# 10258392511/InverseProblemWithDiffusionModel

Hardware: AMD Instinct MI355X
Metric: ALD reconstructions/sec (128x128 complex, R=40, 4-coil) (higher is better)
Workload: dtype f32 (convolutions: operands as two fp16 pieces = 22 significand bits + 2 signs, three fp16 MFMAs per product, fp32 accumulate; every image scaled into fp16's range by an exact power of two from its producer's per-image maxima: any fp32 input, DESIGN.md 4.2); 1 GPU; ACDC-style 128x128 complex SENSE R=40 4-coil ALD reconstruction, NCSNv2Deepest ngf=128 (94.1M params, seeded random init), sigma 348->0.01 x 2311 levels x 3 steps, L2Penalty, denoise; 14 posterior samples = 14 on rank 0 + 13 per further rank (the 105-sample / 8-GPU partition of BASELINE config 3); samples_total=14, samples_this_rank=14, parallelism=sample-sharded x1, hip_graph=True, state_finite=True

## Files before the change

include/ipdm.h:

```cpp
#ifndef IPDM_H
#define IPDM_H

#include <stdint.h>

#ifdef __cplusplus
extern "C" {
#endif

#define IPDM_OK 0
#define IPDM_EINVAL (-1)
#define IPDM_EUNSUPPORTED (-2)

#define IPDM_ACT_NONE 0
#define IPDM_ACT_ELU 1
#define IPDM_ACT_RELU 2
#define IPDM_ACT_LRELU02 3
#define IPDM_ACT_SWISH 4
#define IPDM_ACT_COPY 5

#define IPDM_AMAX_WAYS 8
#define IPDM_AMAX_SLOT 128

#define IPDM_ABI_VERSION 4
int ipdm_abi_version(void);
// ... 190 lines not shown
int ipdm_conv2d_wino_bx3_stats_f32(const float* x, const void* U, const float* bias, const float* residual, float* out,
                                   float* out_act, int act_out, int B, int Cin, int Cout, int H, int W, int dilation,
                                   int pool2, float* stats, const ipdm_conv_ext_t* ext, void* stream);
int ipdm_absmax_f32(const float* x, float* amax , int n_images,
                    int64_t per_image, void* stream);
int64_t ipdm_conv_hx2_weight_bytes(int Cout, int Cin, int k);
int ipdm_conv_hx2_pack_weight(const float* w , void* packed, int Cout,
                              int Cin, int k, void* stream);
int ipdm_conv2d_hx2_f32(const float* x, const void* packed, const float* bias, const float* coef, int act,
                        const float* residual, float* out, float* out_act, int act_out,
                        int B, int Cin, int Cout, int H, int W, int k, int dilation, const ipdm_conv_ext_t* ext, void* stream);
int ipdm_conv3d_hx2_f32(const float* x, const void* packed, const float* bias, const float* coef, int act,
                        const float* residual, float* out, float* out_act, int act_out,
                        int B, int Cin, int Cout, int D, int H, int W, int k, int dilation, const ipdm_conv_ext_t* ext, void* stream);
int ipdm_conv_hx2_splitk_f32(const float* x, const void* packed, const float* bias, const float* coef, int act,
                             const float* residual, float* out, float* out_act, int act_out,
                             int B, int Cin, int Cout, int D, int H, int W, int k, int dilation, int volume, int ksplit,
                             float* work, const ipdm_conv_ext_t* ext, void* stream);
int64_t ipdm_conv_wino_hx2_weight_bytes(int Cout, int Cin);
int ipdm_conv_wino_hx2_pack_weight(const float* w , void* U, int Cout, int Cin, void* stream);
int ipdm_conv2d_wino_hx2_f32(const float* x, const void* U, const float* bias, const float* residual, float* out,
                             float* out_act, int act_out, int B, int Cin, int Cout, int H, int W, int dilation,
                             int pool2, const ipdm_conv_ext_t* ext, void* stream);
int64_t ipdm_conv_wino1d_weight_bytes(int Cout, int Cin);
int ipdm_conv_wino1d_pack_weight(const float* w , void* U, int Cout, int Cin, void* stream);
int ipdm_conv2d_wino1d_supported(int Cin, int Cout, int H, int W);
int64_t ipdm_conv_wino1d_weight_bytes3d(int Cout, int Cin);
int ipdm_conv_wino1d_pack_weight3d(const float* w, void* U, int Cout, int Cin, void* stream);
int ipdm_conv3d_wino1d_supported(int Cin, int Cout, int D, int H, int W);
int ipdm_conv3d_wino1d_f32(const float* x, const void* U, const float* bias, const float* residual, float* out,
                           float* out_act, int act_out, int B, int Cin, int Cout, int D, int H, int W,
                           const ipdm_conv_ext_t* ext, void* stream);
int ipdm_conv2d_wino1d_f32(const float* x, const void* U, const float* bias, const float* coef, int act,
                           const float* residual, float* out, float* out_act, int act_out, int B, int Cin, int Cout, int H,
                           int W, int pool2, const ipdm_conv_ext_t* ext, void* stream);
int ipdm_conv2d_wino1d_stats_partials(int Cin, int Cout, int H, int W);
int ipdm_conv2d_wino1d_stats_f32(const float* x, const void* U, const float* bias, const float* coef, int act,
                                 const float* residual, float* out, float* out_act, int act_out, int B, int Cin, int Cout,
                                 int H, int W, int pool2, float* stats, const ipdm_conv_ext_t* ext, void* stream);
int ipdm_conv2d_wino_hx2_splitk_f32(const float* x, const void* U, const float* bias, const float* residual, float* out,
                                    float* out_act, int act_out, int B, int Cin, int Cout, int H, int W, int dilation,
                                    int ksplit, float* work, const ipdm_conv_ext_t* ext, void* stream);
int ipdm_conv2d_wino_hx2_stats_f32(const float* x, const void* U, const float* bias, const float* residual, float* out,
                                   float* out_act, int act_out, int B, int Cin, int Cout, int H, int W, int dilation,
                                   int pool2, float* stats, const ipdm_conv_ext_t* ext, void* stream);
int ipdm_instnorm_plus_coef_partials_f32(const float* partials, int P, const float* alpha, const float* gamma,
// ... 35 lines not shown
```

inverseproblemwithdiffusionmodel_amd/_lib.py:

```python
import ctypes
import os

import torch
from ctypes import c_char_p, c_float, c_int, c_int64, c_uint64, c_void_p


class ConvExt(ctypes.Structure):
    _fields_ = [("in_amax", c_void_p), ("bias_bstride", c_int), ("out_scale", c_float), ("res_second", c_int),
                ("out_amax", c_void_p), ("act_amax", c_void_p)]


_HERE = os.path.dirname(os.path.abspath(__file__))
LIB_PATH = os.environ.get("IPDM_LIB") or os.path.join(_HERE, "libipdm.so")

P = c_void_p

SIGNATURES = {
    "ipdm_abi_version": [],
    "ipdm_build_arch": [],
    "ipdm_upfirdn2d_f32": [P, P, P] + [c_int] * 14 + [P],
    "ipdm_fused_bias_act_f32": [P, P, P, P, c_int64, c_int, c_int, c_int, c_int, c_float, c_float, P],
    "ipdm_upfirdn2d_f16": [P, P, P] + [c_int] * 14 + [P],
    "ipdm_upfirdn2d_f64": [P, P, P] + [c_int] * 14 + [P],
    "ipdm_fused_bias_act_f16": [P, P, P, P, c_int64, c_int, c_int, c_int, c_int, c_float, c_float, P],
# ... 59 lines not shown
    "ipdm_conv2d_wino_bx3_stats_partials": [c_int, c_int, c_int, c_int, c_int, c_int],
    "ipdm_conv2d_wino_bx3_splitk": [c_int, c_int, c_int, c_int, c_int],
    "ipdm_conv2d_wino_bx3_splitk_f32": [P, P, P, P, P, P, c_int, c_int, c_int, c_int, c_int, c_int, c_int, c_int, P, P, P],
    "ipdm_conv2d_wino_bx3_stats_f32": [P, P, P, P, P, P, c_int, c_int, c_int, c_int, c_int, c_int, c_int, c_int, P, P, P],
    "ipdm_conv_hx2_weight_bytes": [c_int, c_int, c_int],
    "ipdm_conv_hx2_pack_weight": [P, P, c_int, c_int, c_int, P],
    "ipdm_absmax_f32": [P, P, c_int, c_int64, P],
    "ipdm_conv2d_hx2_f32": [P, P, P, P, c_int, P, P, P, c_int] + [c_int] * 7 + [P, P],
    "ipdm_conv3d_hx2_f32": [P, P, P, P, c_int, P, P, P, c_int] + [c_int] * 8 + [P, P],
    "ipdm_conv_hx2_splitk_f32": [P, P, P, P, c_int, P, P, P, c_int] + [c_int] * 10 + [P, P, P],
    "ipdm_conv_wino_hx2_weight_bytes": [c_int, c_int],
    "ipdm_conv_wino1d_weight_bytes": [c_int, c_int],
    "ipdm_conv_wino1d_pack_weight": [P, P, c_int, c_int, P],
    "ipdm_conv2d_wino1d_supported": [c_int, c_int, c_int, c_int],
    "ipdm_conv_wino1d_weight_bytes3d": [c_int, c_int],
    "ipdm_conv_wino1d_pack_weight3d": [P, P, c_int, c_int, P],
    "ipdm_conv3d_wino1d_supported": [c_int, c_int, c_int, c_int, c_int],
    "ipdm_conv3d_wino1d_f32": [P, P, P, P, P, P, c_int, c_int, c_int, c_int, c_int, c_int, c_int, P, P],
    "ipdm_conv2d_wino1d_f32": [P, P, P, P, c_int, P, P, P, c_int, c_int, c_int, c_int, c_int, c_int, c_int, P, P],
    "ipdm_conv2d_wino1d_stats_partials": [c_int, c_int, c_int, c_int],
    "ipdm_conv2d_wino1d_stats_f32": [P, P, P, P, c_int, P, P, P, c_int, c_int, c_int, c_int, c_int, c_int, c_int, P, P, P],
    "ipdm_conv_wino_hx2_pack_weight": [P, P, c_int, c_int, P],
    "ipdm_conv2d_wino_hx2_f32": [P, P, P, P, P, P, c_int, c_int, c_int, c_int, c_int, c_int, c_int, c_int, P, P],
    "ipdm_conv2d_wino_hx2_splitk_f32": [P, P, P, P, P, P, c_int, c_int, c_int, c_int, c_int, c_int, c_int, c_int, P, P, P],
    "ipdm_conv2d_wino_hx2_stats_f32": [P, P, P, P, P, P, c_int, c_int, c_int, c_int, c_int, c_int, c_int, c_int, P, P, P],
    "ipdm_instnorm_plus_coef_partials_f32": [P, c_int, P, P, P, P, c_int, c_int, c_int, P, P],
    "ipdm_cond_instnorm_plus_coef_partials_f32": [P, c_int, P, P, c_int, c_int, P, c_int, c_int, c_int, P, P],
    "ipdm_zero_insert2_f32": [P, P, c_int, c_int, c_int, P],
    "ipdm_subsample2_f32": [P, P, c_int, c_int, c_int, c_int, c_int, c_int, c_int, P],
    "ipdm_in_prelu_fwd_f32": [P, P, P, P, P, c_int, c_int, c_float, P],
    "ipdm_in_prelu_bwd_f32": [P, P, P, P, P, c_int, c_int, P],
    "ipdm_seg_loglh_grad_f32": [P, P, P, c_int, c_int, c_int64, P],
    "ipdm_axpy_sched_f32": [P, P, P, c_int64, P, c_float, c_int64, P],
    "ipdm_magnitude_c64": [P, P, c_int64, P],
    "ipdm_posterior_moments_c64": [P, P, c_int, c_int64, P],
    "ipdm_tv_c64": [P, P, c_int, c_int, c_int, P],
    "ipdm_tv_grad_c64": [P, P, c_int, c_int, c_int, P],
    "ipdm_nrmse_f32": [P, P, P, c_int, c_int64, c_int, P],
    "ipdm_ssim_f32": [P, P, P, c_int, c_int, c_int, c_int, ctypes.c_double, P],
}
_RESTYPES = {"ipdm_build_arch": c_char_p, "ipdm_fft2c_workspace_bytes": c_int64, "ipdm_sense_workspace_bytes": c_int64, "ipdm_conv_bx3_weight_bytes": c_int64,
             "ipdm_conv_wino_bx3_weight_bytes": c_int64, "ipdm_conv_hx2_weight_bytes": c_int64,
             "ipdm_conv_wino_hx2_weight_bytes": c_int64, "ipdm_conv_wino1d_weight_bytes": c_int64, "ipdm_conv_wino1d_weight_bytes3d": c_int64}

IPDM_EINVAL = -1
IPDM_EUNSUPPORTED = -2
# ... 39 lines not shown
```

inverseproblemwithdiffusionmodel_amd/csrc/conv_wino_bx3.hip:

```cpp
#include "conv_kernel.h"

namespace ipdm_conv {

namespace {

constexpr int X_KC = 16;
constexpr int X_CO = 64;
constexpr int X_TX = 16, X_TY = 4;
constexpr int X_TILES = X_TX * X_TY;
constexpr int X_V_ELEMS = 16 * X_KC * X_TILES;
constexpr int X_RR = 2 * X_TY + 2, X_RC = 2 * X_TX + 2;
constexpr int X_RCH = 384;
constexpr int X_R_ELEMS = 32 * 256;
constexpr size_t X_LDS_BYTES = (2 * (size_t)X_V_ELEMS + X_R_ELEMS) * sizeof(float);

__global__ __launch_bounds__(256) void wino_bx3_weight_kernel(const float* __restrict__ w, unsigned short* __restrict__ out,
                                                              int Cout, int Cin, int n_cc, int n_ct) {
  const float G[4][3] = {{1.f, 0.f, 0.f}, {0.5f, 0.5f, 0.5f}, {0.5f, -0.5f, 0.5f}, {0.f, 0.f, 1.f}};
  const int64_t total = (int64_t)16 * n_cc * n_ct * 512;
  for (int64_t i = (int64_t)blockIdx.x * 256 + threadIdx.x; i < total; i += (int64_t)gridDim.x * 256) {
    const int q = (int)(i & 7), r = (int)((i >> 3) & 31), h = (int)((i >> 8) & 1);
    const int64_t rest = i >> 9;
    const int ct = (int)(rest % n_ct);
    const int cc = (int)((rest / n_ct) % n_cc);
// ... 479 lines not shown
              const float e1 = a.act_out == IPDM_ACT_ELU ? fast_elu(y1v) : ipdm_act(y1v, a.act_out);
              amx_a = fmaxf(amx_a, fmaxf(fabsf(e0), fabsf(e1)));
              *reinterpret_cast<float2*>(a.out_act + o) = make_float2(e0, e1);
            }
          }
        }
      }
    }
  }
  if (a.amax_out) ipdm_amax_commit(amx_o, a.amax_out + (size_t)b * IPDM_AMAX_SLOT, wave);
  if (a.amax_act) ipdm_amax_commit(amx_a, a.amax_act + (size_t)b * IPDM_AMAX_SLOT, wave);
  if (a.dbg) {
    __builtin_amdgcn_s_waitcnt(0);
    const unsigned long long t3 = __builtin_amdgcn_s_memtime();
    if (tid == 0) {
      unsigned long long* d4 = a.dbg + (size_t)blockIdx.x * 4;
      d4[0] = t0; d4[1] = t1; d4[2] = t2; d4[3] = t3;
    }
  }
}


template <bool HX, int TX, int TY, bool CO_MAJOR, bool DMA4, bool POOL = false, bool STATS = false, bool KSP = false, bool POLY = false,
          bool CO32 = false>
__global__ __launch_bounds__(512) void conv_wino_bx3_wide_kernel(ConvArgs a, int total_tiles) {
  constexpr int NPC = HX ? 2 : 3;
  constexpr int FRAG = 64 * NPC;
  constexpr int NC = CO32 ? 1 : 2;
  static_assert(!CO32 || (HX && TX == 8 && TY == 8 && DMA4 && !POOL && !STATS && !KSP && !POLY), "CO32: the plain 8 x 8 form");
  static_assert(!POLY || (TX == 8 && TY == 8 && DMA4 && !POOL && !STATS && !KSP), "POLY: the 8 x 8 form, plain epilogue");
  constexpr int PPW = 24, PPH = 17;
  constexpr int QC = POLY ? PPW / 4 : TX / 2 + 2, RC4 = 4 * QC;
  constexpr int QN = POLY ? PPH * QC : (2 * TY + 2) * QC;
  constexpr int NI = (X_KC * QN + 63) / 64;
  static_assert(NI >= 24 && NI <= 32 && NI * 256 <= X_R_ELEMS, "quad image fits the raw stage; pieces 0..23 exist");
  constexpr bool WPRIV = HX && DMA4;
  static_assert(!WPRIV || 2 * QN <= 256, "a wave's two channels fit four DMA instructions");
  static_assert(TX * TY == X_TILES, "64 tiles per workgroup");
  constexpr int RC = 2 * TX + 2, RR = 2 * TY + 2;
  static_assert(RC * RR <= X_RCH, "raw region fits its LDS slot");
  extern __shared__ __align__(16) float lds[];
  unsigned long long t0 = 0, t1 = 0, t2 = 0;
  if (a.dbg) t0 = __builtin_amdgcn_s_memtime();
  const int tid = threadIdx.x;
  const int lane = tid & 63;
  const int wave = __builtin_amdgcn_readfirstlane(tid >> 6);
  const int h = lane >> 5, j = lane & 31;
  const int HW = a.H * a.W;
  const int n_cc = a.Cin / X_KC, n_ct = a.Cout / 32;
  const int n_chunks = KSP ? n_cc / a.ksplit : n_cc;
  const int p0 = 2 * wave;

  const int S = gridDim.x / 8;
  const int xcd = blockIdx.x % 8, slot = blockIdx.x / 8;
  const int q = total_tiles / 8, r8 = total_tiles % 8;
  const int x_start = xcd < r8 ? xcd * (q + 1) : r8 * (q + 1) + (xcd - r8) * q;
  const int x_end = x_start + q + (xcd < r8 ? 1 : 0);
#ifdef IPDM_WBX3_RUNS
  constexpr bool RUNS = true;
#else
  constexpr bool RUNS = false;
// ... 9 lines not shown
    Geo g;
    g.ks = 0;
    g.c0 = 0;
    int n_px = total_tiles / a.co_tiles;
    if constexpr (KSP) {
      g.ks = L % a.ksplit;
      L /= a.ksplit;
      n_px /= a.ksplit;
      g.c0 = g.ks * n_chunks;
    }
    g.co_tile = CO_MAJOR ? L / n_px : L % a.co_tiles;
    int t = CO_MAJOR ? L % n_px : L / a.co_tiles;
    const int tx = t % a.tiles_x;
    t /= a.tiles_x;
    g.y0 = (t % a.tiles_y) * (2 * TY);
    g.x0 = tx * (2 * TX);
    g.b = t / a.tiles_y;
    return g;
  };

  const __amdgpu_buffer_rsrc_t x_rsrc = __builtin_amdgcn_make_buffer_rsrc(
      const_cast<float*>(a.x), 0, (int)((size_t)a.B * a.Cin * HW * 4), 0x00020000);
  float* const rs = lds + 2 * X_V_ELEMS;
  const int mytile = tid & 63;

  int dma_off[DMA4 ? 4 : 6];
  int dma_b = 0;
  [[maybe_unused]] int dma_c0 = 0;
  auto dma_piece = [&](int k) { return wave + 8 * k < NI ? wave + 8 * k : wave + 8 * (k - 1); };
  auto set_dma_geo = [&](const Geo& g) {
    dma_b = g.b;
    if constexpr (KSP) dma_c0 = g.c0;
    if constexpr (DMA4) {
#pragma unroll
      for (int k = 0; k < 4; ++k) {
        const int e = (WPRIV ? k : dma_piece(k)) * 64 + lane;
        const int cl = e / QN, qq = e - cl * QN;
        const int cin = WPRIV ? 2 * wave + cl : cl;
        const int rr = qq / QC, qc = qq - rr * QC;
        const int gy = POLY ? (rr < 16 ? rr : -1) : g.y0 - 1 + rr, gx0 = g.x0 - 4 + 4 * qc;
        const bool ok = e < (WPRIV ? 2 : X_KC) * QN && gy >= 0 && gy < a.H && gx0 >= 0 && gx0 < a.W;
        dma_off[k] = ok ? (cin * HW + gy * a.W + gx0) * 4 : 0x40000000;
      }
    } else {
#pragma unroll
      for (int k = 0; k < 6; ++k) {
        const int e = k * 64 + lane;
        const int rr = e / RC, c = e - rr * RC;
        const int gy = g.y0 - 1 + rr, gx = g.x0 - 1 + c;
        const bool ok = e < RR * RC && gy >= 0 && gy < a.H && gx >= 0 && gx < a.W;
        dma_off[k] = ok ? (gy * a.W + gx) * 4 : 0x40000000;
      }
    }
  };
  auto issue_dma = [&](int chunk) {
    if constexpr (KSP) chunk += dma_c0;
    if constexpr (DMA4) {
      [[maybe_unused]] const int soff = (int)(((size_t)dma_b * a.Cin + chunk * X_KC) * HW * 4);
#pragma unroll
      for (int k = 0; k < 4; ++k) {
#if defined(__HIP_DEVICE_COMPILE__)
        __builtin_amdgcn_raw_ptr_buffer_load_lds(
            x_rsrc, (__attribute__((address_space(3))) void*)(rs + (WPRIV ? wave * 4 + k : dma_piece(k)) * 256), 16, dma_off[k],
            soff, 0, 0);
#endif
      }
    } else {
#pragma unroll
      for (int cl = 0; cl < 2; ++cl) {
        const int kc = 2 * wave + cl;
        const int soff = (int)(((size_t)dma_b * a.Cin + chunk * X_KC + kc) * HW * 4);
#pragma unroll
        for (int k = 0; k < 6; ++k)
          __builtin_amdgcn_raw_ptr_buffer_load_lds(x_rsrc, (__attribute__((address_space(3))) void*)(rs + kc * X_RCH + k * 64), 4,
                                                   dma_off[k], soff, 0, 0);
      }
    }
  };
  float dreg[16];
  const int pd = POLY ? a.dil : 1;
  auto tile_origin = [&](int tl, int& py, int& px) {
    const int tws = a.W / (2 * pd), ths = a.H / (2 * pd);
    const int txx = tl % tws;
    int r = tl / tws;
    const int tyy = r % ths;
    r /= ths;
    py = pd * (2 * tyy) + r / pd;
    px = pd * (2 * txx) + r % pd;
  };
  [[maybe_unused]] int prow[4], pcol[4];
  if constexpr (POLY) {
    int py, px;
    tile_origin(mytile, py, px);
#pragma unroll
    for (int e = 0; e < 4; ++e) {
      const int gy = py + pd * (e - 1), gx = px + pd * (e - 1);
      prow[e] = (gy >= 0 && gy < a.H ? gy : 16) * PPW;
      pcol[e] = gx >= 0 && gx < a.W ? gx + 4 : 0;
    }
  }
  const int r_lane = DMA4 ? (2 * (mytile / TX)) * RC4 + 2 * (mytile % TX) + 2 : (2 * (mytile / TX)) * RC + 2 * (mytile % TX);
  auto read_patch_to = [&](float (&dreg)[16], int kc) {
    if constexpr (POLY) {
      const float* rp = WPRIV ? rs + wave * 1024 + (kc & 1) * (QN * 4) : rs + kc * (QN * 4);
#pragma unroll
      for (int rr = 0; rr < 4; ++rr)
#pragma unroll
        for (int cc = 0; cc < 4; ++cc) dreg[rr * 4 + cc] = rp[prow[rr] + pcol[cc]];
    } else if constexpr (DMA4) {
      const float* rp = (WPRIV ? rs + wave * 1024 + (kc & 1) * (QN * 4) : rs + kc * (QN * 4)) + r_lane;
      const int txl = mytile % TX;
// ... 62 lines not shown
  [[maybe_unused]] float hx_in = HX_WINO_PRESCALE, hx_out = 1.f;
  auto hx_scales_of = [&](int b, float& s_in, float& s_out) {
    s_in = HX_WINO_PRESCALE;
    s_out = 1.f;
    if constexpr (HX) {
      if (a.in_amax) {
        float sd, si;
        hx_dynamic_scale(ipdm_amax_read(a.in_amax + (size_t)b * IPDM_AMAX_SLOT), sd, si);
        s_in = HX_WINO_PRESCALE * sd;
        s_out = si;
      }
    }
  };
  auto store_pair = [&](float* st, const float (&va)[16], const float (&vb)[16], auto p_lo, auto p_hi) {
    unsigned* vs = reinterpret_cast<unsigned*>(st) + wave * X_TILES + mytile;
#pragma unroll
    for (int p = decltype(p_lo)::value; p < decltype(p_hi)::value; ++p) {
      unsigned hp, lp;
      split2_pk_scaled(va[p], vb[p], hx_in, hp, lp);
      vs[(p * 2 + 0) * (8 * X_TILES)] = hp;
      vs[(p * 2 + 1) * (8 * X_TILES)] = lp;
    }
  };
  auto stage_chunk = [&](float* st) {
    if constexpr (HX) {
      float va[16], vb[16];
      read_patch_to(va, 2 * wave);
      transform(va);
      read_patch_to(vb, 2 * wave + 1);
      transform(vb);
      store_pair(st, va, vb, std::integral_constant<int, 0>{}, std::integral_constant<int, 16>{});
    } else {
      read_patch(2 * wave);
      store_patch(st, 2 * wave);
      read_patch(2 * wave + 1);
      store_patch(st, 2 * wave + 1);
    }
  };

  const uint4* wq = reinterpret_cast<const uint4*>(a.wt);
  const size_t pos_stride = (size_t)n_cc * n_ct * FRAG;
  auto load_A = [&](uint4 (&fr)[NC][NPC], int p, int cc, int co_tile) {
    const uint4* base = wq + (size_t)p * pos_stride + ((size_t)cc * n_ct + co_tile * NC) * FRAG + lane;
#pragma unroll
    for (int c = 0; c < NC; ++c)
#pragma unroll
      for (int s = 0; s < NPC; ++s) fr[c][s] = base[c * FRAG + s * 64];
  };
  const int b_lane = (8 * h) * X_TILES + j;
  auto load_B = [&](float (&raw)[8], const float* cur, int pi, int tg) {
    const float* bp = cur + (p0 + pi) * (X_KC * X_TILES) + tg * 32 + b_lane;
#pragma unroll
    for (int qq = 0; qq < 8; ++qq) raw[qq] = bp[qq * X_TILES];
  };
  auto load_Bh = [&](uint4 (&fr)[2], const float* cur, int pi, int tg) {
    const unsigned* bp = reinterpret_cast<const unsigned*>(cur) + (p0 + pi) * (X_KC * X_TILES) + (4 * h) * X_TILES + tg * 32 + j;
#pragma unroll
    for (int s = 0; s < 2; ++s)
      fr[s] = make_uint4(bp[s * 8 * X_TILES], bp[(s * 8 + 1) * X_TILES], bp[(s * 8 + 2) * X_TILES], bp[(s * 8 + 3) * X_TILES]);
  };

  f32x16 acc[2][NC][2];
  auto zero_acc = [&]() {
#pragma unroll
    for (int i = 0; i < 4 * NC; ++i)
#pragma unroll
      for (int rr = 0; rr < 16; ++rr) acc[i / (2 * NC)][(i >> 1) % NC][i & 1][rr] = 0.f;
  };
  zero_acc();

  Geo cur_g = geo_of(tile);
  uint4 afr[2][NC][NPC];
  load_A(afr[0], p0, cur_g.c0, cur_g.co_tile);
  if constexpr (WPRIV) load_A(afr[1], p0 + 1, cur_g.c0, cur_g.co_tile);
  hx_scales_of(cur_g.b, hx_in, hx_out);
  set_dma_geo(cur_g);
  auto lds_barrier = [&]() {
    __builtin_amdgcn_sched_barrier(0);
    __builtin_amdgcn_s_waitcnt(0xC07F);
    __builtin_amdgcn_s_barrier();
    asm volatile("" ::: "memory");
    __builtin_amdgcn_sched_barrier(0);
  };
  issue_dma(0);
  __builtin_amdgcn_s_waitcnt(0);
  __syncthreads();
  stage_chunk(lds);
  __syncthreads();
  issue_dma(1);
  __builtin_amdgcn_s_waitcnt(0);
// ... 23 lines not shown
#define IPDM_TE(k)
#endif
  while (true) {
    const int next_tile = tile + t_step;
    const bool has_next = next_tile < t_end;
    const Geo next_g = geo_of(has_next ? next_tile : tile);
    for (int ch = 0; ch < n_chunks; ++ch, ++g) {
#ifdef IPDM_WBX3_TRACE
      const bool trace_now = g == n_chunks + 2;
#endif
      IPDM_TR(0);
      const float* cur = lds + (g & 1) * X_V_ELEMS;
      float* nxt = lds + ((g + 1) & 1) * X_V_ELEMS;
      const bool dma_next = ch + 2 >= n_chunks;
      const int dma_chunk = dma_next ? ch + 2 - n_chunks : ch + 2;
      if (ch + 2 == n_chunks) set_dma_geo(next_g);
      const bool a_next = ch + 1 >= n_chunks;
      const int a_chunk = a_next ? next_g.c0 : cur_g.c0 + ch + 1;
      const int a_cot = a_next ? next_g.co_tile : cur_g.co_tile;
      if constexpr (HX) {
        [[maybe_unused]] float unused_out;
        if (a_next && next_g.b != cur_g.b) hx_scales_of(next_g.b, hx_in, unused_out);
      }
      if constexpr (WPRIV) {
        uint4 bsh[2][2];
        float va[16], vb[16];
        __builtin_amdgcn_s_waitcnt(0x0F74);
        read_patch_to(va, 2 * wave);
        read_patch_to(vb, 2 * wave + 1);
        load_Bh(bsh[0], cur, 0, 0);
        __builtin_amdgcn_sched_barrier(0);
        __builtin_amdgcn_s_waitcnt(0xC07F);
        IPDM_TR(5);
        issue_dma(dma_chunk);
        __builtin_amdgcn_sched_barrier(0);
        static_for<4>([&](auto sc) {
          constexpr int st = decltype(sc)::value;
          constexpr int pi = st >> 1, tg = st & 1;
          if constexpr (st < 3) load_Bh(bsh[(st + 1) & 1], cur, (st + 1) >> 1, (st + 1) & 1);
          if constexpr (st == 0) transform(va);
          if constexpr (st == 1) transform(vb);
          if constexpr (st == 2) {
            store_pair(nxt, va, vb, std::integral_constant<int, 0>{}, std::integral_constant<int, 8>{});
            load_A(afr[0], p0, a_chunk, a_cot);
          }
          if constexpr (st == 3) store_pair(nxt, va, vb, std::integral_constant<int, 8>{}, std::integral_constant<int, 16>{});
          const f16x8 bh = __builtin_bit_cast(f16x8, bsh[st & 1][0]), bl = __builtin_bit_cast(f16x8, bsh[st & 1][1]);
// ... 151 lines not shown
    if (a.dbg) t2 = __builtin_amdgcn_s_memtime();

    float* ms = lds + ((g - 1) & 1) * X_V_ELEMS;
    IPDM_TE(0);
    const int etile = tid & 31, ecg = tid >> 5;
    const int co0 = cur_g.co_tile * (CO32 ? 32 : X_CO);
    constexpr int NR = POOL ? 1 : 2;
    constexpr bool AHEAD = TX == 16;
    float2 resv[AHEAD ? 2 : 1][2][NR];
    float biasv[AHEAD ? 2 : 1][2];
    [[maybe_unused]] float scalev[AHEAD ? 2 : 1][2];
    const float* const scale_p = HX ? reinterpret_cast<const float*>(wq + 16 * pos_stride) : a.wt;
    [[maybe_unused]] const int oH = POOL ? a.H >> 1 : a.H, oW = POOL ? a.W >> 1 : a.W;
    [[maybe_unused]] constexpr int rstep = POOL ? 1 : 2;
    [[maybe_unused]] const size_t tile_base =
        ((KSP ? (size_t)cur_g.ks * a.B * a.Cout * HW : 0) +
         ((size_t)cur_g.b * a.Cout + co0) * ((size_t)oH * oW) + (size_t)(POOL ? cur_g.y0 >> 1 : cur_g.y0) * oW +
         (POOL ? cur_g.x0 >> 1 : cur_g.x0)) * 4;
    [[maybe_unused]] unsigned eoff4 = 4u * (unsigned)((ecg * 2) * (oH * oW) + rstep * (etile / TX) * oW + rstep * (etile % TX));
    asm volatile("" : "+v"(eoff4));
    [[maybe_unused]] auto boff = [&](int c, int tg, int i, int ii) -> unsigned {
      return 4u * (unsigned)((c * 32 + i) * (oH * oW) + (rstep * (tg * 32 / TX) + ii) * oW) + eoff4;
    };
    auto out_index = [&](int c, int tg, int i, int ii) -> size_t {
      int py, px;
      tile_origin(tg * 32 + etile, py, px);
      return ((size_t)cur_g.b * a.Cout + co0 + c * 32 + ecg * 2 + i) * HW + (size_t)(py + pd * ii) * a.W + px;
    };
    auto in_range = [&](int tg) {
      if constexpr (POLY) return true;
      const int T = tg * 32 + etile;
      return cur_g.y0 + 2 * (T / TX) < a.H && cur_g.x0 + 2 * (T % TX) < a.W;
    };
    const bool has_res = a.residual != nullptr, has_bias = a.bias != nullptr;
    const float* const res_p = has_res ? a.residual : a.wt;
    const float* const bias_p = has_bias ? a.bias : a.wt;
    [[maybe_unused]] const char* const res_b = reinterpret_cast<const char*>(res_p) + (has_res ? tile_base : 0);
    [[maybe_unused]] char* const out_b = reinterpret_cast<char*>(a.out) + tile_base;
    [[maybe_unused]] char* const act_b = reinterpret_cast<char*>(a.out_act) + tile_base;
    auto prefetch = [&](auto rc) {
      constexpr int rnd = decltype(rc)::value;
      constexpr int c = rnd >> 1, tg = rnd & 1, bf = AHEAD ? rnd & 1 : 0;
      const bool res_ok = has_res && in_range(tg);
#pragma unroll
      for (int i = 0; i < 2; ++i) {
        biasv[bf][i] = bias_p[has_bias ? cur_g.b * a.bias_bstride + co0 + c * 32 + ecg * 2 + i : 0];
        if constexpr (HX) scalev[bf][i] = scale_p[co0 + c * 32 + ecg * 2 + i] * hx_out;
#pragma unroll
        for (int ii = 0; ii < NR; ++ii) {
          if constexpr (POLY) {
            const size_t o = res_ok ? out_index(c, tg, i, ii) : 0;
            resv[bf][i][ii] = make_float2(res_p[o], res_p[o + (res_ok ? pd : 0)]);
          } else {
            const unsigned ob = res_ok ? boff(c, tg, i, ii) : 0u;
            if constexpr (POOL) resv[bf][i][ii] = make_float2(*reinterpret_cast<const float*>(res_b + ob), 0.f);
            else resv[bf][i][ii] = *reinterpret_cast<const float2*>(res_b + ob);
          }
        }
      }
    };
    if constexpr (!KSP) {
      if (cur_g.b != pend_b) {
        flush_amax();
        pend_b = cur_g.b;
        pend_o = pend_a = 0u;
      }
    }
    if constexpr (AHEAD) prefetch(std::integral_constant<int, 0>{});
    [[maybe_unused]] float amx_o = 0.f, amx_a = 0.f;
    static_for<2 * NC>([&](auto rc) {
      constexpr int rnd = decltype(rc)::value;
      constexpr int c = rnd >> 1, tg = rnd & 1, bf = AHEAD ? rnd & 1 : 0;
      if constexpr (!AHEAD) prefetch(rc);
#pragma unroll
      for (int pi = 0; pi < 2; ++pi)
#pragma unroll
        for (int rr = 0; rr < 16; ++rr) {
          const int col = (rr & 3) + 8 * (rr >> 2) + 4 * h;
          ms[((p0 + pi) * 32 + col) * 32 + j] = acc[pi][c][tg][rr];
          acc[pi][c][tg][rr] = 0.f;
        }
      IPDM_TE(1 + 4 * rnd);
      __syncthreads();
      IPDM_TE(2 + 4 * rnd);
      if constexpr (AHEAD && rnd < 2 * NC - 1) prefetch(std::integral_constant<int, rnd + 1>{});
      constexpr int NSV = POOL ? 1 : 4;
      [[maybe_unused]] float sv[2][NSV];
      if constexpr (STATS) {
#pragma unroll
        for (int i = 0; i < 2; ++i)
#pragma unroll
          for (int k = 0; k < NSV; ++k) sv[i][k] = 0.f;
      }
      if constexpr (rnd == 1) { IPDM_TF(0); }
      if (in_range(tg)) {
#pragma unroll
        for (int i = 0; i < 2; ++i) {
          const int cl = ecg * 2 + i;
          float m[16];
#pragma unroll
          for (int p = 0; p < 16; ++p) m[p] = ms[(p * 32 + cl) * 32 + etile];
          float tt[2][4];
#pragma unroll
          for (int qq = 0; qq < 4; ++qq) {
            tt[0][qq] = m[0 * 4 + qq] + m[1 * 4 + qq] + m[2 * 4 + qq];
            tt[1][qq] = m[1 * 4 + qq] - m[2 * 4 + qq] - m[3 * 4 + qq];
          }
#ifdef IPDM_WBX3_TRACE
// ... 165 lines not shown


bool x_small(const ConvArgs& a) { return a.W < 32 || a.dil > 1; }
bool x_small_dma(const ConvArgs& a) {
  static int min_pairs = -1;
  if (min_pairs < 0) {
    const char* e = getenv("IPDM_WBX3_SMALL_MIN");
    min_pairs = e ? atoi(e) : 160;
  }
  return a.dil == 1 && a.W <= 16 && a.H <= 16 && a.W % 2 == 0 && a.H % 2 == 0 && a.Cin >= 2 * X_KC &&
         (int64_t)a.B * (a.Cout / X_CO) >= min_pairs;
}

bool x_co32(const ConvArgs& a) {
  static int enabled = -1;
  if (enabled < 0) {
    const char* e = getenv("IPDM_WBX3_CO32");
    enabled = e ? atoi(e) : 1;
  }
  return enabled && a.hx && a.dil == 1 && a.W <= 16 && a.H <= 16 && a.W % 4 == 0 && a.H % 2 == 0 && a.Cin >= 2 * X_KC &&
         a.Cout < 512 && !a.pool2 && !a.stats;
}

int wino_persist() {
  static int persist = -1;
  if (persist < 0) {
    const char* e = getenv("IPDM_WBX3_PERSIST");
    persist = e ? atoi(e) : 1;
  }
  return persist;
}

int cus_per_xcd() {
  static int n = 0;
  if (!n) {
    int dev = 0, v = 0;
    if (hipGetDevice(&dev) == hipSuccess &&
        hipDeviceGetAttribute(&v, hipDeviceAttributeMultiprocessorCount, dev) == hipSuccess && v >= 8)
      n = v / 8;
    else
      n = 32;
  }
  return n;
}

}
// ... 2 lines not shown
  if (!(ks == 3 && a.D == 1 && a.Cin % X_KC == 0 && a.Cout % X_CO == 0 && !a.coef && a.act == IPDM_ACT_NONE)) return false;
  if (a.dil < 1 || a.dil > 4) return false;
  if ((size_t)a.B * a.Cin * a.H * a.W * 4 >= (x_small(a) ? 0x1fffffffull : 0x3fffffffull)) return false;
  if (x_small(a)) return a.H % (2 * a.dil) == 0 && a.W % (2 * a.dil) == 0 && (a.H * a.W) / 4 >= 32;
  return a.H % 2 == 0 && a.W % 2 == 0 && a.H >= 8;
}

bool x_poly(const ConvArgs& a) {
  static int enabled = -1;
  if (enabled < 0) {
    const char* e = getenv("IPDM_WBX3_POLY");
    enabled = e ? atoi(e) : 1;
  }
  return enabled && wino_persist() && a.dil > 1 && a.H == 16 && a.W == 16 && 16 % (2 * a.dil) == 0 && a.Cin >= 2 * X_KC &&
         !a.pool2 && !a.stats && (reinterpret_cast<uintptr_t>(a.x) & 15) == 0;
}

template <bool HXV>
static int conv_wino_bx3_launch_t(ConvArgs a, hipStream_t s) {
  if (x_poly(a)) {
    a.tiles_x = a.tiles_y = 1;
    a.co_tiles = a.Cout / X_CO;
    const int64_t nblk = (int64_t)a.B * a.co_tiles;
    static bool poly_attr = false;
    if (!poly_attr) {
      (void)hipFuncSetAttribute(reinterpret_cast<const void*>(conv_wino_bx3_wide_kernel<HXV, 8, 8, true, true, false, false, false, true>),
                                hipFuncAttributeMaxDynamicSharedMemorySize, X_LDS_BYTES);
      poly_attr = true;
    }
    const int per_xcd = (int)((nblk + 7) / 8);
    const int S = per_xcd < cus_per_xcd() ? per_xcd : cus_per_xcd();
    hipLaunchKernelGGL((conv_wino_bx3_wide_kernel<HXV, 8, 8, true, true, false, false, false, true>), dim3((unsigned)(8 * S)),
                       dim3(512), X_LDS_BYTES, s, a, (int)nblk);
    return ipdm_launch_status();
  }
  const bool small = x_small(a);
  if (HXV && small && wino_persist() && x_co32(a) && (reinterpret_cast<uintptr_t>(a.x) & 15) == 0) {
    a.tiles_x = (a.W + 15) / 16;
    a.tiles_y = (a.H + 15) / 16;
    a.co_tiles = a.Cout / 32;
    const int64_t nblk = (int64_t)a.B * a.tiles_x * a.tiles_y * a.co_tiles;
    if (nblk > 0x7fffffff) return IPDM_EUNSUPPORTED;
    static bool co32_attr = false;
    if (!co32_attr) {
      (void)hipFuncSetAttribute(reinterpret_cast<const void*>(conv_wino_bx3_wide_kernel<true, 8, 8, true, true, false, false, false, false, true>),
                                hipFuncAttributeMaxDynamicSharedMemorySize, X_LDS_BYTES);
      co32_attr = true;
    }
    const int per_xcd = (int)((nblk + 7) / 8);
    const int S = per_xcd < cus_per_xcd() ? per_xcd : cus_per_xcd();
    hipLaunchKernelGGL((conv_wino_bx3_wide_kernel<true, 8, 8, true, true, false, false, false, false, true>), dim3((unsigned)(8 * S)),
                       dim3(512), X_LDS_BYTES, s, a, (int)nblk);
    return ipdm_launch_status();
  }
  const bool small_dma = small && wino_persist() && x_small_dma(a);
  if (a.pool2 && (small || !wino_persist() || a.Cin < 2 * X_KC || a.H % 2 || a.W % 2)) return IPDM_EUNSUPPORTED;
  if (small_dma) {
    a.tiles_x = (a.W + 15) / 16;
    a.tiles_y = (a.H + 15) / 16;
  } else if (small) {
    a.tiles_x = ((a.H * a.W) / 4 + X_TILES - 1) / X_TILES;
    a.tiles_y = 1;
  } else {
    a.tiles_x = (a.W + 2 * X_TX - 1) / (2 * X_TX);
    a.tiles_y = (a.H + 2 * X_TY - 1) / (2 * X_TY);
  }
  a.co_tiles = a.Cout / X_CO;
  const int64_t nblk = (int64_t)a.B * a.tiles_x * a.tiles_y * a.co_tiles;
  if (nblk > 0x7fffffff) return IPDM_EUNSUPPORTED;
  static bool attr_set = false;
  if (!attr_set) {
// ... 170 lines not shown
  a.act_out = act_out; a.B = B; a.Cin = Cin; a.Cout = Cout; a.H = H; a.W = W; a.dil = dilation; a.act = IPDM_ACT_NONE;
  a.D = 1; a.kd = 1; a.tiles_x = a.tiles_y = a.co_tiles = 0; a.dbg = conv_debug_stamps();
  a.pool2 = pool2 ? 1 : 0;
  a.stats = stats;
  a.hx = hx;
  conv_apply_ext(a, ext, hx);
  if (!wino_bx3_ok(a, 3)) return IPDM_EUNSUPPORTED;
  return conv_wino_bx3_launch(a, ipdm_stream(stream));
}

extern "C" int ipdm_conv2d_wino_bx3_f32(const float* x, const void* U, const float* bias, const float* residual,
                                        float* out, float* out_act, int act_out, int B, int Cin, int Cout, int H, int W,
                                        int dilation, int pool2, const ipdm_conv_ext_t* ext, void* stream) {
  return wino_bx3_entry(x, U, bias, residual, out, out_act, act_out, B, Cin, Cout, H, W, dilation, pool2, nullptr, stream, 0, ext);
}

extern "C" int ipdm_conv2d_wino_bx3_splitk(int Cin, int Cout, int H, int W, int dilation) {
  ConvArgs a;
  a.coef = nullptr; a.act = IPDM_ACT_NONE; a.dil = dilation; a.D = 1; a.Cin = Cin; a.Cout = Cout; a.H = H; a.W = W; a.B = 1;
  if (!wino_bx3_ok(a, 3)) return 1;
  return wino_bx3_ksplit_for(Cin, Cout, H, W, dilation);
}

static int wino_bx3_splitk_entry(const float* x, const void* U, const float* bias, const float* residual, float* out,
                                 float* out_act, int act_out, int B, int Cin, int Cout, int H, int W, int dilation, int ksplit,
                                 float* work, void* stream, int hx, const ipdm_conv_ext_t* ext = nullptr) {
  IPDM_REQUIRE(B >= 0 && Cin > 0 && Cout > 0 && H > 0 && W > 0 && dilation >= 1 && ksplit >= 2);
  if (B == 0) return IPDM_OK;
  IPDM_REQUIRE(x && U && work && (out || out_act) && x != out && x != out_act);
  IPDM_REQUIRE(B <= 65535 || !ext || (!ext->out_amax && !ext->act_amax));
  ConvArgs a;
  a.x = x; a.wt = (const float*)U; a.bias = bias; a.coef = nullptr; a.residual = residual; a.out = out; a.out_act = out_act;
  a.act_out = act_out; a.B = B; a.Cin = Cin; a.Cout = Cout; a.H = H; a.W = W; a.dil = dilation; a.act = IPDM_ACT_NONE;
  a.D = 1; a.kd = 1; a.tiles_x = a.tiles_y = a.co_tiles = 0; a.dbg = nullptr;
  a.hx = hx;
  conv_apply_ext(a, ext, hx);
  if (!wino_bx3_ok(a, 3)) return IPDM_EUNSUPPORTED;
  return conv_wino_bx3_launch_ksplit(a, ksplit, work, ipdm_stream(stream));
}

extern "C" int ipdm_conv2d_wino_bx3_splitk_f32(const float* x, const void* U, const float* bias, const float* residual,
                                               float* out, float* out_act, int act_out, int B, int Cin, int Cout, int H,
                                               int W, int dilation, int ksplit, float* work, const ipdm_conv_ext_t* ext, void* stream) {
  return wino_bx3_splitk_entry(x, U, bias, residual, out, out_act, act_out, B, Cin, Cout, H, W, dilation, ksplit, work, stream, 0, ext);
}

// ... 42 lines not shown
```

inverseproblemwithdiffusionmodel_amd/ops.py:

```python
import ctypes
import os

import torch

from . import _lib
from ._lib import call, P

ACT_NONE, ACT_ELU, ACT_RELU, ACT_LRELU02, ACT_SWISH = 0, 1, 2, 3, 4
ACT_COPY = 5
CONV_TRACE = None

ACT_CODES = {"none": ACT_NONE, None: ACT_NONE, "elu": ACT_ELU, "relu": ACT_RELU, "lrelu": ACT_LRELU02,
             "swish": ACT_SWISH}


def _gpu(t, dtype=None, name="tensor"):
    if not isinstance(t, torch.Tensor) or not t.is_cuda:
        raise RuntimeError(f"ipdm: {name} must be a GPU tensor (the HIP path has no CPU fallback); got "
                           f"{getattr(t, 'device', type(t))}")
    if dtype is not None and t.dtype != dtype:
        raise TypeError(f"ipdm: {name} must be {dtype}, got {t.dtype}")
    return t if t.is_contiguous() else t.contiguous()


# ... 1278 lines not shown
        CONV_TRACE.append(dict(B=B, Cin=Cin, Cout=Cout, H=H, W=W, k=3, dil=dilation, wino=True, bx3=True, fmt=U.fmt, res=residual is not None,
                               n_out=int(raw) + int(want_act), pool2=bool(pool2), wino1d=one_d, stats=part is not None, e0=e0, e1=e1))
    tag_amax(out, slot_o)
    tag_amax(out_act, slot_a)
    return (out, out_act) if want_act else out


WBX3_CO32 = os.environ.get("IPDM_WBX3_CO32", "1") != "0"


def wino_bx3_pays(Cin, Cout, H, W, dilation=1, B=None):
    if W <= 16 and dilation == 1:
        if wino_bx3_splitk(Cin, Cout, H, W, dilation) > 1:
            return True
        if H > 16 or Cout < 512 or Cin < 32:
            return False
    return conv_wino_bx3_supported(Cin, Cout, H, W, dilation)


def wino_bx3_splitk(Cin, Cout, H, W, dilation=1):
    return int(_lib.lib.ipdm_conv2d_wino_bx3_splitk(int(Cin), int(Cout), int(H), int(W), int(dilation)))


def wino_bx3_max_batch(Cin, H, W, dilation=1):
    reach = 0x1fffffff if (W < 32 or dilation > 1) else 0x3fffffff
    return max(1, (reach - 1) // (Cin * H * W * 4))


def adam_ascent(x, g, m, v, lr, step, betas=(0.9, 0.999), eps=1e-8):
    for t, n in ((x, "x"), (g, "g"), (m, "m"), (v, "v")):
        _inplace_operand(t, torch.float32, n)
        if t.numel() != x.numel():
            raise ValueError(f"adam_ascent: {n} does not match x")
    call("ipdm_adam_ascent_f32", _ptr(x), _ptr(g), _ptr(m), _ptr(v), x.numel(), float(lr), float(betas[0]), float(betas[1]),
         float(eps), int(step), _stream())
    _written(x, m, v)
    return x
```

Baseline: 0.1263 reconstructions/s.

## Add half-tile Winograd form for 16x16 convs to double workgroup count

Adds a HALF variant of the wide Winograd hx2 kernel that handles an 8x4 tile group (32 tiles) per workgroup for 16x16 feature maps. Each wave transforms one channel patch and trades halves across lanes with permlane32_swap, with its own MFMA/DMA schedule. This doubles the number of workgroups for these small layers so more CUs are used, at the cost of less weight reuse per workgroup. It also replaces divisions in the polyphase tile_origin with shifts, makes the max-LDS attribute per-device, and adds a form-query API.

Result: faster. 0.1295 reconstructions/s (median of 6 runs) (+2.6%).

```diff
diff --git a/include/ipdm.h b/include/ipdm.h
--- a/include/ipdm.h
+++ b/include/ipdm.h
@@ -236,6 +236,11 @@
 int ipdm_conv2d_wino_hx2_f32(const float* x, const void* U, const float* bias, const float* residual, float* out,
                              float* out_act, int act_out, int B, int Cin, int Cout, int H, int W, int dilation,
                              int pool2, const ipdm_conv_ext_t* ext, void* stream);
+#define IPDM_WINO_FORM_OTHER 0
+#define IPDM_WINO_FORM_CO32 1
+#define IPDM_WINO_FORM_HALF 2
+#define IPDM_WINO_FORM_POLY 3
+int ipdm_conv2d_wino_hx2_form(int Cin, int Cout, int H, int W, int dilation);
 int64_t ipdm_conv_wino1d_weight_bytes(int Cout, int Cin);
 int ipdm_conv_wino1d_pack_weight(const float* w , void* U, int Cout, int Cin, void* stream);
 int ipdm_conv2d_wino1d_supported(int Cin, int Cout, int H, int W);
diff --git a/inverseproblemwithdiffusionmodel_amd/_lib.py b/inverseproblemwithdiffusionmodel_amd/_lib.py
--- a/inverseproblemwithdiffusionmodel_amd/_lib.py
+++ b/inverseproblemwithdiffusionmodel_amd/_lib.py
@@ -105,6 +105,7 @@
     "ipdm_conv2d_wino1d_stats_f32": [P, P, P, P, c_int, P, P, P, c_int, c_int, c_int, c_int, c_int, c_int, c_int, P, P, P],
     "ipdm_conv_wino_hx2_pack_weight": [P, P, c_int, c_int, P],
     "ipdm_conv2d_wino_hx2_f32": [P, P, P, P, P, P, c_int, c_int, c_int, c_int, c_int, c_int, c_int, c_int, P, P],
+    "ipdm_conv2d_wino_hx2_form": [c_int] * 5,
     "ipdm_conv2d_wino_hx2_splitk_f32": [P, P, P, P, P, P, c_int, c_int, c_int, c_int, c_int, c_int, c_int, c_int, P, P, P],
     "ipdm_conv2d_wino_hx2_stats_f32": [P, P, P, P, P, P, c_int, c_int, c_int, c_int, c_int, c_int, c_int, c_int, P, P, P],
     "ipdm_instnorm_plus_coef_partials_f32": [P, c_int, P, P, P, P, c_int, c_int, c_int, P, P],
diff --git a/inverseproblemwithdiffusionmodel_amd/csrc/conv_wino_bx3.hip b/inverseproblemwithdiffusionmodel_amd/csrc/conv_wino_bx3.hip
--- a/inverseproblemwithdiffusionmodel_amd/csrc/conv_wino_bx3.hip
+++ b/inverseproblemwithdiffusionmodel_amd/csrc/conv_wino_bx3.hip
@@ -525,21 +525,24 @@
 
 
 template <bool HX, int TX, int TY, bool CO_MAJOR, bool DMA4, bool POOL = false, bool STATS = false, bool KSP = false, bool POLY = false,
-          bool CO32 = false>
+          bool CO32 = false, bool HALF = false>
 __global__ __launch_bounds__(512) void conv_wino_bx3_wide_kernel(ConvArgs a, int total_tiles) {
   constexpr int NPC = HX ? 2 : 3;
   constexpr int FRAG = 64 * NPC;
   constexpr int NC = CO32 ? 1 : 2;
   static_assert(!CO32 || (HX && TX == 8 && TY == 8 && DMA4 && !POOL && !STATS && !KSP && !POLY), "CO32: the plain 8 x 8 form");
   static_assert(!POLY || (TX == 8 && TY == 8 && DMA4 && !POOL && !STATS && !KSP), "POLY: the 8 x 8 form, plain epilogue");
+  static_assert(!HALF || (HX && TX == 8 && TY == 4 && DMA4 && !POOL && !STATS && !KSP && !POLY && !CO32), "HALF: the plain 8 x 4 form");
+  constexpr int NTG = HALF ? 1 : 2;
+  constexpr int NDMA = HALF ? 2 : 4;
   constexpr int PPW = 24, PPH = 17;
   constexpr int QC = POLY ? PPW / 4 : TX / 2 + 2, RC4 = 4 * QC;
   constexpr int QN = POLY ? PPH * QC : (2 * TY + 2) * QC;
   constexpr int NI = (X_KC * QN + 63) / 64;
-  static_assert(NI >= 24 && NI <= 32 && NI * 256 <= X_R_ELEMS, "quad image fits the raw stage; pieces 0..23 exist");
+  static_assert(HALF || (NI >= 24 && NI <= 32 && NI * 256 <= X_R_ELEMS), "quad image fits the raw stage; pieces 0..23 exist");
   constexpr bool WPRIV = HX && DMA4;
-  static_assert(!WPRIV || 2 * QN <= 256, "a wave's two channels fit four DMA instructions");
-  static_assert(TX * TY == X_TILES, "64 tiles per workgroup");
+  static_assert(!WPRIV || 2 * QN <= 64 * NDMA, "a wave's two channels fit its DMA instructions");
+  static_assert(TX * TY * 2 == X_TILES * NTG, "32 tiles per tile group");
   constexpr int RC = 2 * TX + 2, RR = 2 * TY + 2;
   static_assert(RC * RR <= X_RCH, "raw region fits its LDS slot");
   extern __shared__ __align__(16) float lds[];
@@ -595,7 +598,7 @@
   const __amdgpu_buffer_rsrc_t x_rsrc = __builtin_amdgcn_make_buffer_rsrc(
       const_cast<float*>(a.x), 0, (int)((size_t)a.B * a.Cin * HW * 4), 0x00020000);
   float* const rs = lds + 2 * X_V_ELEMS;
-  const int mytile = tid & 63;
+  const int mytile = HALF ? tid & 31 : tid & 63;
 
   int dma_off[DMA4 ? 4 : 6];
   int dma_b = 0;
@@ -606,7 +609,7 @@
     if constexpr (KSP) dma_c0 = g.c0;
     if constexpr (DMA4) {
 #pragma unroll
-      for (int k = 0; k < 4; ++k) {
+      for (int k = 0; k < NDMA; ++k) {
         const int e = (WPRIV ? k : dma_piece(k)) * 64 + lane;
         const int cl = e / QN, qq = e - cl * QN;
         const int cin = WPRIV ? 2 * wave + cl : cl;
@@ -631,7 +634,7 @@
     if constexpr (DMA4) {
       [[maybe_unused]] const int soff = (int)(((size_t)dma_b * a.Cin + chunk * X_KC) * HW * 4);
 #pragma unroll
-      for (int k = 0; k < 4; ++k) {
+      for (int k = 0; k < NDMA; ++k) {
 #if defined(__HIP_DEVICE_COMPILE__)
         __builtin_amdgcn_raw_ptr_buffer_load_lds(
             x_rsrc, (__attribute__((address_space(3))) void*)(rs + (WPRIV ? wave * 4 + k : dma_piece(k)) * 256), 16, dma_off[k],
@@ -652,14 +655,11 @@
   };
   float dreg[16];
   const int pd = POLY ? a.dil : 1;
+  const int pls = pd == 4 ? 1 : pd == 2 ? 2 : 3;
   auto tile_origin = [&](int tl, int& py, int& px) {
-    const int tws = a.W / (2 * pd), ths = a.H / (2 * pd);
-    const int txx = tl % tws;
-    int r = tl / tws;
-    const int tyy = r % ths;
-    r /= ths;
-    py = pd * (2 * tyy) + r / pd;
-    px = pd * (2 * txx) + r % pd;
+    const int txx = tl & ((1 << pls) - 1), tyy = (tl >> pls) & ((1 << pls) - 1), r = tl >> (2 * pls);
+    py = pd * (2 * tyy) + (r >> (3 - pls));
+    px = pd * (2 * txx) + (r & (pd - 1));
   };
   [[maybe_unused]] int prow[4], pcol[4];
   if constexpr (POLY) {
@@ -768,8 +768,34 @@
       vs[(p * 2 + 1) * (8 * X_TILES)] = lp;
     }
   };
+  [[maybe_unused]] auto trade_halves = [&](const float (&v)[16], float (&vp)[8][2]) {
+#pragma unroll
+    for (int p = 0; p < 8; ++p) {
+#if defined(__HIP_DEVICE_COMPILE__)
+      const auto r = __builtin_amdgcn_permlane32_swap(__builtin_bit_cast(unsigned, v[p]), __builtin_bit_cast(unsigned, v[p + 8]), false, false);
+      vp[p][0] = __builtin_bit_cast(float, (unsigned)r[0]);
+      vp[p][1] = __builtin_bit_cast(float, (unsigned)r[1]);
+#endif
+    }
+  };
+  [[maybe_unused]] auto store_half = [&](float* st, const float (&vp)[8][2]) {
+    unsigned* vs = reinterpret_cast<unsigned*>(st) + wave * X_TILES + mytile + (8 * h) * 2 * (8 * X_TILES);
+#pragma unroll
+    for (int p = 0; p < 8; ++p) {
+      unsigned hp, lp;
+      split2_pk_scaled(vp[p][0], vp[p][1], hx_in, hp, lp);
+      vs[(p * 2 + 0) * (8 * X_TILES)] = hp;
+      vs[(p * 2 + 1) * (8 * X_TILES)] = lp;
+    }
+  };
   auto stage_chunk = [&](float* st) {
-    if constexpr (HX) {
+    if constexpr (HALF) {
+      float va[16], vp[8][2];
+      read_patch_to(va, h);
+      transform(va);
+      trade_halves(va, vp);
+      store_half(st, vp);
+    } else if constexpr (HX) {
       float va[16], vb[16];
       read_patch_to(va, 2 * wave);
       transform(va);
@@ -806,12 +832,12 @@
       fr[s] = make_uint4(bp[s * 8 * X_TILES], bp[(s * 8 + 1) * X_TILES], bp[(s * 8 + 2) * X_TILES], bp[(s * 8 + 3) * X_TILES]);
   };
 
-  f32x16 acc[2][NC][2];
+  f32x16 acc[2][NC][NTG];
   auto zero_acc = [&]() {
 #pragma unroll
-    for (int i = 0; i < 4 * NC; ++i)
-#pragma unroll
-      for (int rr = 0; rr < 16; ++rr) acc[i / (2 * NC)][(i >> 1) % NC][i & 1][rr] = 0.f;
+    for (int i = 0; i < 2 * NC * NTG; ++i)
+#pragma unroll
+      for (int rr = 0; rr < 16; ++rr) acc[i / (NTG * NC)][(i / NTG) % NC][i % NTG][rr] = 0.f;
   };
   zero_acc();
 
@@ -881,7 +907,49 @@
         [[maybe_unused]] float unused_out;
         if (a_next && next_g.b != cur_g.b) hx_scales_of(next_g.b, hx_in, unused_out);
       }
-      if constexpr (WPRIV) {
+      if constexpr (HALF) {
+        uint4 bsh[2][2];
+        float va[16], vp[8][2];
+        __builtin_amdgcn_s_waitcnt(0x0F74);
+        read_patch_to(va, h);
+        load_Bh(bsh[0], cur, 0, 0);
+        __builtin_amdgcn_sched_barrier(0);
+        __builtin_amdgcn_s_waitcnt(0xC07F);
+        IPDM_TR(5);
+        issue_dma(dma_chunk);
+        __builtin_amdgcn_sched_barrier(0);
+        static_for<2>([&](auto sc) {
+          constexpr int pi = decltype(sc)::value;
+          if constexpr (pi == 0) {
+            load_Bh(bsh[1], cur, 1, 0);
+            transform(va);
+            trade_halves(va, vp);
+          } else {
+            store_half(nxt, vp);
+            load_A(afr[0], p0, a_chunk, a_cot);
+          }
+          const f16x8 bh = __builtin_bit_cast(f16x8, bsh[pi][0]), bl = __builtin_bit_cast(f16x8, bsh[pi][1]);
+#pragma unroll
+          for (int c = 0; c < NC; ++c) {
+            f32x16 v = acc[pi][c][0];
+            v = __builtin_amdgcn_mfma_f32_32x32x16_f16(__builtin_bit_cast(f16x8, afr[pi][c][1]), bh, v, 0, 0, 0);
+            v = __builtin_amdgcn_mfma_f32_32x32x16_f16(__builtin_bit_cast(f16x8, afr[pi][c][0]), bl, v, 0, 0, 0);
+            v = __builtin_amdgcn_mfma_f32_32x32x16_f16(__builtin_bit_cast(f16x8, afr[pi][c][0]), bh, v, 0, 0, 0);
+            acc[pi][c][0] = v;
+          }
+          if constexpr (pi == 0) __builtin_amdgcn_sched_group_barrier(0x100, 8, 0);
+          if constexpr (pi == 1) __builtin_amdgcn_sched_group_barrier(0x020, 4, 0);
+#pragma unroll
+          for (int i = 0; i < 6; ++i) {
+            __builtin_amdgcn_sched_group_barrier(0x008, 1, 0);
+            __builtin_amdgcn_sched_group_barrier(0x006, pi == 0 ? 10 : 8, 0);
+            if constexpr (pi == 1) __builtin_amdgcn_sched_group_barrier(0x200, 3, 0);
+          }
+          __builtin_amdgcn_sched_barrier(0);
+          IPDM_TR(1 + pi);
+        });
+        load_A(afr[1], p0 + 1, a_chunk, a_cot);
+      } else if constexpr (WPRIV) {
         uint4 bsh[2][2];
         float va[16], vb[16];
         __builtin_amdgcn_s_waitcnt(0x0F74);
@@ -1079,10 +1147,13 @@
     [[maybe_unused]] auto boff = [&](int c, int tg, int i, int ii) -> unsigned {
       return 4u * (unsigned)((c * 32 + i) * (oH * oW) + (rstep * (tg * 32 / TX) + ii) * oW) + eoff4;
     };
+    const size_t poly_base = ((size_t)cur_g.b * a.Cout + co0) * HW;
+    [[maybe_unused]] int etile_p = etile;
+    if constexpr (POLY) asm volatile("" : "+v"(etile_p));
     auto out_index = [&](int c, int tg, int i, int ii) -> size_t {
       int py, px;
-      tile_origin(tg * 32 + etile, py, px);
-      return ((size_t)cur_g.b * a.Cout + co0 + c * 32 + ecg * 2 + i) * HW + (size_t)(py + pd * ii) * a.W + px;
+      tile_origin(tg * 32 + etile_p, py, px);
+      return poly_base + (unsigned)((c * 32 + ecg * 2 + i) * HW + (py + pd * ii) * a.W + px);
     };
     auto in_range = [&](int tg) {
       if constexpr (POLY) return true;
@@ -1097,7 +1168,7 @@
     [[maybe_unused]] char* const act_b = reinterpret_cast<char*>(a.out_act) + tile_base;
     auto prefetch = [&](auto rc) {
       constexpr int rnd = decltype(rc)::value;
-      constexpr int c = rnd >> 1, tg = rnd & 1, bf = AHEAD ? rnd & 1 : 0;
+      constexpr int c = rnd / NTG, tg = rnd % NTG, bf = AHEAD ? rnd & 1 : 0;
       const bool res_ok = has_res && in_range(tg);
 #pragma unroll
       for (int i = 0; i < 2; ++i) {
@@ -1125,9 +1196,9 @@
     }
     if constexpr (AHEAD) prefetch(std::integral_constant<int, 0>{});
     [[maybe_unused]] float amx_o = 0.f, amx_a = 0.f;
-    static_for<2 * NC>([&](auto rc) {
+    static_for<NTG * NC>([&](auto rc) {
       constexpr int rnd = decltype(rc)::value;
-      constexpr int c = rnd >> 1, tg = rnd & 1, bf = AHEAD ? rnd & 1 : 0;
+      constexpr int c = rnd / NTG, tg = rnd % NTG, bf = AHEAD ? rnd & 1 : 0;
       if constexpr (!AHEAD) prefetch(rc);
 #pragma unroll
       for (int pi = 0; pi < 2; ++pi)
@@ -1140,7 +1211,7 @@
       IPDM_TE(1 + 4 * rnd);
       __syncthreads();
       IPDM_TE(2 + 4 * rnd);
-      if constexpr (AHEAD && rnd < 2 * NC - 1) prefetch(std::integral_constant<int, rnd + 1>{});
+      if constexpr (AHEAD && rnd < NTG * NC - 1) prefetch(std::integral_constant<int, rnd + 1>{});
       constexpr int NSV = POOL ? 1 : 4;
       [[maybe_unused]] float sv[2][NSV];
       if constexpr (STATS) {
@@ -1352,6 +1423,24 @@
          a.Cout < 512 && !a.pool2 && !a.stats;
 }
 
+bool x_half(const ConvArgs& a) {
+  static int enabled = -1;
+  if (enabled < 0) {
+    const char* e = getenv("IPDM_WBX3_HALF");
+    enabled = e ? atoi(e) : 1;
+  }
+  return enabled && x_co32(a) && a.W == 16 && a.H == 16;
+}
+
+template <typename K>
+void set_max_lds_once(K kernel, bool (&done)[64]) {
+  int dev = 0;
+  if (hipGetDevice(&dev) != hipSuccess || dev < 0 || dev >= 64) dev = 0;
+  if (done[dev]) return;
+  (void)hipFuncSetAttribute(reinterpret_cast<const void*>(kernel), hipFuncAttributeMaxDynamicSharedMemorySize, X_LDS_BYTES);
+  done[dev] = true;
+}
+
 int wino_persist() {
   static int persist = -1;
   if (persist < 0) {
@@ -1400,12 +1489,8 @@
     a.tiles_x = a.tiles_y = 1;
     a.co_tiles = a.Cout / X_CO;
     const int64_t nblk = (int64_t)a.B * a.co_tiles;
-    static bool poly_attr = false;
-    if (!poly_attr) {
-      (void)hipFuncSetAttribute(reinterpret_cast<const void*>(conv_wino_bx3_wide_kernel<HXV, 8, 8, true, true, false, false, false, true>),
-                                hipFuncAttributeMaxDynamicSharedMemorySize, X_LDS_BYTES);
-      poly_attr = true;
-    }
+    static bool poly_attr[64] = {};
+    set_max_lds_once(conv_wino_bx3_wide_kernel<HXV, 8, 8, true, true, false, false, false, true>, poly_attr);
     const int per_xcd = (int)((nblk + 7) / 8);
     const int S = per_xcd < cus_per_xcd() ? per_xcd : cus_per_xcd();
     hipLaunchKernelGGL((conv_wino_bx3_wide_kernel<HXV, 8, 8, true, true, false, false, false, true>), dim3((unsigned)(8 * S)),
@@ -1414,17 +1499,27 @@
   }
   const bool small = x_small(a);
   if (HXV && small && wino_persist() && x_co32(a) && (reinterpret_cast<uintptr_t>(a.x) & 15) == 0) {
+    if (x_half(a)) {
+      a.tiles_x = 1;
+      a.tiles_y = 2;
+      a.co_tiles = a.Cout / X_CO;
+      const int64_t nblk = (int64_t)a.B * 2 * a.co_tiles;
+      if (nblk > 0x7fffffff) return IPDM_EUNSUPPORTED;
+      static bool half_attr[64] = {};
+      set_max_lds_once(conv_wino_bx3_wide_kernel<true, 8, 4, true, true, false, false, false, false, false, true>, half_attr);
+      const int per_xcd = (int)((nblk + 7) / 8);
+      const int S = per_xcd < cus_per_xcd() ? per_xcd : cus_per_xcd();
+      hipLaunchKernelGGL((conv_wino_bx3_wide_kernel<true, 8, 4, true, true, false, false, false, false, false, true>), dim3((unsigned)(8 * S)),
+                         dim3(512), X_LDS_BYTES, s, a, (int)nblk);
+      return ipdm_launch_status();
+    }
     a.tiles_x = (a.W + 15) / 16;
     a.tiles_y = (a.H + 15) / 16;
     a.co_tiles = a.Cout / 32;
     const int64_t nblk = (int64_t)a.B * a.tiles_x * a.tiles_y * a.co_tiles;
     if (nblk > 0x7fffffff) return IPDM_EUNSUPPORTED;
-    static bool co32_attr = false;
-    if (!co32_attr) {
-      (void)hipFuncSetAttribute(reinterpret_cast<const void*>(conv_wino_bx3_wide_kernel<true, 8, 8, true, true, false, false, false, false, true>),
-                                hipFuncAttributeMaxDynamicSharedMemorySize, X_LDS_BYTES);
-      co32_attr = true;
-    }
+    static bool co32_attr[64] = {};
+    set_max_lds_once(conv_wino_bx3_wide_kernel<true, 8, 8, true, true, false, false, false, false, true>, co32_attr);
     const int per_xcd = (int)((nblk + 7) / 8);
     const int S = per_xcd < cus_per_xcd() ? per_xcd : cus_per_xcd();
     hipLaunchKernelGGL((conv_wino_bx3_wide_kernel<true, 8, 8, true, true, false, false, false, false, true>), dim3((unsigned)(8 * S)),
@@ -1641,6 +1736,16 @@
   return wino_bx3_ksplit_for(Cin, Cout, H, W, dilation);
 }
 
+extern "C" int ipdm_conv2d_wino_hx2_form(int Cin, int Cout, int H, int W, int dilation) {
+  ConvArgs a;
+  a.x = nullptr; a.coef = nullptr; a.act = IPDM_ACT_NONE; a.dil = dilation; a.D = 1; a.Cin = Cin; a.Cout = Cout; a.H = H; a.W = W;
+  a.B = 1; a.hx = 1; a.pool2 = 0; a.stats = nullptr;
+  if (Cin <= 0 || Cout <= 0 || H <= 0 || W <= 0 || dilation < 1 || !wino_bx3_ok(a, 3)) return IPDM_EUNSUPPORTED;
+  if (x_poly(a)) return IPDM_WINO_FORM_POLY;
+  if (x_small(a) && wino_persist() && x_co32(a)) return x_half(a) ? IPDM_WINO_FORM_HALF : IPDM_WINO_FORM_CO32;
+  return IPDM_WINO_FORM_OTHER;
+}
+
 static int wino_bx3_splitk_entry(const float* x, const void* U, const float* bias, const float* residual, float* out,
                                  float* out_act, int act_out, int B, int Cin, int Cout, int H, int W, int dilation, int ksplit,
                                  float* work, void* stream, int hx, const ipdm_conv_ext_t* ext = nullptr) {
diff --git a/inverseproblemwithdiffusionmodel_amd/ops.py b/inverseproblemwithdiffusionmodel_amd/ops.py
--- a/inverseproblemwithdiffusionmodel_amd/ops.py
+++ b/inverseproblemwithdiffusionmodel_amd/ops.py
@@ -1324,6 +1324,14 @@
     return int(_lib.lib.ipdm_conv2d_wino_bx3_splitk(int(Cin), int(Cout), int(H), int(W), int(dilation)))
 
 
+WINO_FORM_OTHER, WINO_FORM_CO32, WINO_FORM_HALF, WINO_FORM_POLY = 0, 1, 2, 3
+
+
+def wino_hx2_form(Cin, Cout, H, W, dilation=1):
+    f = int(_lib.lib.ipdm_conv2d_wino_hx2_form(int(Cin), int(Cout), int(H), int(W), int(dilation)))
+    return None if f < 0 else f
+
+
 def wino_bx3_max_batch(Cin, H, W, dilation=1):
     reach = 0x1fffffff if (W < 32 or dilation > 1) else 0x3fffffff
     return max(1, (reach - 1) // (Cin * H * W * 4))
```
